# videolan/dav1d

Hardware: NVIDIA H100
Metric: Mpixels/s (higher is better)
Workload: dtype u8/i16->i32

## Files before the change

dav1d_b200/csrc/loopfilter.cu:

```cuda
#include "host_util.h"

namespace b200 {

template <bool HBD> struct LfMem {
    typename Bd<HBD>::pixel *p; ptrdiff_t sb;
    B200_DEV int get(int i) const { return p[i * sb]; }
    B200_DEV void set(int i, int v) { p[i * sb] = (typename Bd<HBD>::pixel)v; }
};
template <bool HBD, class Acc>
B200_DEV void lf_line_acc(Acc &px, int E, int I, int H, int wd, int bdmax)
{
    const int b8 = HBD ? (32 - __clz(bdmax)) - 8 : 0;
    const int F = 1 << b8;
    E <<= b8; I <<= b8; H <<= b8;
    const int p1 = px.get(-2), p0 = px.get(-1), q0 = px.get(0), q1 = px.get(1);
    int fm = iabs(p1 - p0) <= I && iabs(q1 - q0) <= I && iabs(p0 - q0) * 2 + (iabs(p1 - q1) >> 1) <= E;
    int p2 = 0, q2 = 0, p3 = 0, q3 = 0;
    if (wd > 4) {
        p2 = px.get(-3); q2 = px.get(2);
        fm &= iabs(p2 - p1) <= I && iabs(q2 - q1) <= I;
        if (wd > 6) {
            p3 = px.get(-4); q3 = px.get(3);
            fm &= iabs(p3 - p2) <= I && iabs(q3 - q2) <= I;
        }
    }
    if (!fm) return;
    int flat8in = 0;
    if (wd >= 6) flat8in = iabs(p2 - p0) <= F && iabs(p1 - p0) <= F && iabs(q1 - q0) <= F && iabs(q2 - q0) <= F;
    if (wd >= 8) flat8in &= iabs(p3 - p0) <= F && iabs(q3 - q0) <= F;
    if (wd >= 16) {
        const int p6 = px.get(-7), p5 = px.get(-6), p4 = px.get(-5), q4 = px.get(4), q5 = px.get(5), q6 = px.get(6);
        const int flat8out = iabs(p6 - p0) <= F && iabs(p5 - p0) <= F && iabs(p4 - p0) <= F &&
                             iabs(q4 - q0) <= F && iabs(q5 - q0) <= F && iabs(q6 - q0) <= F;
        if (flat8out & flat8in) {
            int s = p6 * 7 + p5 * 2 + p4 * 2 + p3 + p2 + p1 + p0 + q0 + 8;
            px.set(-6, (s >> 4)); s += -2 * p6 + p3 + q1;
            px.set(-5, (s >> 4)); s += -p6 - p5 + p2 + q2;
            px.set(-4, (s >> 4)); s += -p6 - p4 + p1 + q3;
            px.set(-3, (s >> 4)); s += -p6 - p3 + p0 + q4;
            px.set(-2, (s >> 4)); s += -p6 - p2 + q0 + q5;
            px.set(-1, (s >> 4)); s += -p6 - p1 + q1 + q6;
            px.set(0, (s >> 4)); s += -p5 - p0 + q2 + q6;
            px.set(1, (s >> 4)); s += -p4 - q0 + q3 + q6;
            px.set(2, (s >> 4)); s += -p3 - q1 + q4 + q6;
            px.set(3, (s >> 4)); s += -p2 - q2 + q5 + q6;
            px.set(4, (s >> 4)); s += -p1 - q3 + q6 + q6;
            px.set(5, (s >> 4));
            return;
        }
    }
    if (wd >= 8 && flat8in) {
        px.set(-3, ((p3 + p3 + p3 + 2 * p2 + p1 + p0 + q0 + 4) >> 3));
        px.set(-2, ((p3 + p3 + p2 + 2 * p1 + p0 + q0 + q1 + 4) >> 3));
        px.set(-1, ((p3 + p2 + p1 + 2 * p0 + q0 + q1 + q2 + 4) >> 3));
        px.set(0, ((p2 + p1 + p0 + 2 * q0 + q1 + q2 + q3 + 4) >> 3));
        px.set(1, ((p1 + p0 + q0 + 2 * q1 + q2 + q3 + q3 + 4) >> 3));
        px.set(2, ((p0 + q0 + q1 + 2 * q2 + q3 + q3 + q3 + 4) >> 3));
    } else if (wd == 6 && flat8in) {
        px.set(-2, ((p2 + 2 * p2 + 2 * p1 + 2 * p0 + q0 + 4) >> 3));
        px.set(-1, ((p2 + 2 * p1 + 2 * p0 + 2 * q0 + q1 + 4) >> 3));
        px.set(0, ((p1 + 2 * p0 + 2 * q0 + 2 * q1 + q2 + 4) >> 3));
        px.set(1, ((p0 + 2 * q0 + 2 * q1 + 2 * q2 + q2 + 4) >> 3));
    } else {
        const int lo = -128 * (1 << b8), hi = 128 * (1 << b8) - 1;
        const bool hev = iabs(p1 - p0) > H || iabs(q1 - q0) > H;
        int f = hev ? iclip(p1 - q1, lo, hi) : 0;
        f = iclip(3 * (q0 - p0) + f, lo, hi);
        const int f1 = imin(f + 4, hi) >> 3, f2 = imin(f + 3, hi) >> 3;
        px.set(-1, iclip(p0 + f2, 0, bdmax));
        px.set(0, iclip(q0 - f1, 0, bdmax));
        if (!hev) {
            const int g = (f1 + 1) >> 1;
            px.set(-2, iclip(p1 + g, 0, bdmax));
            px.set(1, iclip(q1 - g, 0, bdmax));
        }
    }
}

template <bool HBD>
B200_DEV void lf_line(typename Bd<HBD>::pixel *p, ptrdiff_t sb, int E, int I, int H, int wd, int bdmax)
{
    LfMem<HBD> m{ p, sb };
    lf_line_acc<HBD>(m, E, I, H, wd, bdmax);
}

B200_DEV int lf_width(const B200Av1Filter &m, int plane, int dir, int b, int a, int ss_a)
{
    if (plane == 0) {
        const int half = a >> 4, bit = a & 15;
        if ((m.filter_y[dir][b][2][half] >> bit) & 1) return 16;
        if ((m.filter_y[dir][b][1][half] >> bit) & 1) return 8;
        if ((m.filter_y[dir][b][0][half] >> bit) & 1) return 4;
        return 0;
    }
    const int hs = 16 >> ss_a;
    const int half = a >= hs, bit = a - half * hs;
    if ((m.filter_uv[dir][b][1][half] >> bit) & 1) return 6;
    if ((m.filter_uv[dir][b][0][half] >> bit) & 1) return 4;
    return 0;
}

template <bool HBD>
__global__ void __launch_bounds__(256) lf_cols_kernel(const __grid_constant__ B200LfFrame f, int bdmax, int ya4, int yb4)
{
    B200_PDL_ENTRY();
    typedef typename Bd<HBD>::pixel pixel;
    const int plane = blockIdx.z;
    if (plane ? !f.filter_uv : !f.filter_y) return;
    const int ssh = plane ? f.ss_hor : 0, ssv = plane ? f.ss_ver : 0;
    const int x4 = blockIdx.x * 32 + threadIdx.x;
    const int y4 = (ya4 >> ssv) + blockIdx.y * 8 + threadIdx.y;
    const int pw4 = (f.w4 + ssh) >> ssh, ph4 = imin((f.h4 + ssv) >> ssv, (yb4 + ssv) >> ssv);
    if (x4 >= pw4 || x4 == 0 || y4 >= ph4) return;
    const int sbx = x4 >> (5 - ssh), xi = x4 & ((32 >> ssh) - 1);
    const int sby = y4 >> (5 - ssv), yi = y4 & ((32 >> ssv) - 1);
    const B200Av1Filter &m = f.mask[sby * f.sb128w + sbx];
    const int wd = lf_width(m, plane, 0, xi, yi, ssv);
    if (!wd) return;
    const uint8_t (*l)[4] = f.level + (ptrdiff_t)y4 * f.b4_stride + x4;
    const int c = plane == 0 ? 0 : plane + 1;
    const int L = l[0][c] ? l[0][c] : l[-1][c];
    if (!L) return;
    const int E = f.lut.e[L], I = f.lut.i[L];
    pixel *p = (pixel *)f.pic + f.plane_off[plane] + (ptrdiff_t)(y4 * 4) * f.stride[plane] + x4 * 4;
#pragma unroll 1
    for (int k = 0; k < 4; k++, p += f.stride[plane]) lf_line<HBD>(p, 1, E, I, L >> 4, wd, bdmax);
}

template <bool HBD>
__global__ void __launch_bounds__(256) lf_rows_kernel(const __grid_constant__ B200LfFrame f, int bdmax, int ya4, int yb4)
{
    B200_PDL_ENTRY();
    typedef typename Bd<HBD>::pixel pixel;
    const int plane = blockIdx.z;
    if (plane ? !f.filter_uv : !f.filter_y) return;
    const int ssh = plane ? f.ss_hor : 0, ssv = plane ? f.ss_ver : 0;
    const int x = blockIdx.x * 128 + threadIdx.x;
    const int y4 = (ya4 >> ssv) + blockIdx.y * 2 + threadIdx.y;
    const int pw4 = (f.w4 + ssh) >> ssh, ph4 = imin((f.h4 + ssv) >> ssv, (yb4 + ssv) >> ssv);
    if (x >= pw4 * 4 || y4 >= ph4 || y4 == 0) return;
    const int x4 = x >> 2, sbx = x4 >> (5 - ssh), xi = x4 & ((32 >> ssh) - 1);
    const int sby = y4 >> (5 - ssv), yi = y4 & ((32 >> ssv) - 1);
    const B200Av1Filter &m = f.mask[sby * f.sb128w + sbx];
    const int wd = lf_width(m, plane, 1, yi, xi, ssh);
    if (!wd) return;
    const uint8_t (*l)[4] = f.level + (ptrdiff_t)y4 * f.b4_stride + x4;
    const int c = plane == 0 ? 1 : plane + 1;
    const int L = l[0][c] ? l[0][c] : l[-f.b4_stride][c];
    if (!L) return;
    pixel *p = (pixel *)f.pic + f.plane_off[plane] + (ptrdiff_t)(y4 * 4) * f.stride[plane] + x;
    lf_line<HBD>(p, f.stride[plane], f.lut.e[L], f.lut.i[L], L >> 4, wd, bdmax);
}

struct LfSbArgs {
    uint32_t mask[3];
    uint8_t cur[32], prev[32];
    B200FilterLUT lut;
    int plane_class, dir, n_units, stride;
};
template <bool HBD>
__global__ void lf_sb_kernel(typename Bd<HBD>::pixel *dst, LfSbArgs a, int bdmax)
{
    const int line = blockIdx.x * blockDim.x + threadIdx.x;
    if (line >= a.n_units * 4) return;
    const int u = line >> 2;
    int wd = 0;
    if (a.plane_class) wd = (a.mask[1] >> u) & 1 ? 6 : ((a.mask[0] >> u) & 1 ? 4 : 0);
    else wd = (a.mask[2] >> u) & 1 ? 16 : ((a.mask[1] >> u) & 1 ? 8 : ((a.mask[0] >> u) & 1 ? 4 : 0));
    if (!wd) return;
    const int L = a.cur[u] ? a.cur[u] : a.prev[u];
    if (!L) return;
    typename Bd<HBD>::pixel *p = a.dir ? dst + 8 * a.stride + line : dst + (ptrdiff_t)line * a.stride + 8;
    lf_line<HBD>(p, a.dir ? a.stride : 1, a.lut.e[L], a.lut.i[L], L >> 4, wd, bdmax);
}

int lf_frame_rows(int bdmax, const B200LfFrame *f, int ya4, int yb4, cudaStream_t stream)
{
    if (int r = check_bdmax(bdmax, "b200_lf_frame")) return r;
    if (!f->filter_y) return 0;
    ya4 = imax(ya4, 0); yb4 = imin(yb4, f->h4);
    if (yb4 <= ya4) return 0;
    if ((ya4 & 1) || ((yb4 & 1) && yb4 != f->h4)) { b200_set_error("b200_lf_frame: odd band boundary"); return -2; }
    const int w4 = f->w4, n4 = yb4 - ya4;
    if (int r = launch_hbd(bdmax, Launch::pdl, dim3((w4 + 31) / 32, (n4 + 7) / 8, 3), dim3(32, 8), 0, stream,
                           [&](auto hbd) { return std::make_tuple(lf_cols_kernel<hbd>, *f, bdmax, ya4, yb4); }))
        return r;
    return launch_hbd(bdmax, Launch::pdl, dim3((w4 * 4 + 127) / 128, (n4 + 1) / 2, 3), dim3(128, 2), 0, stream,
                      [&](auto hbd) { return std::make_tuple(lf_rows_kernel<hbd>, *f, bdmax, ya4, yb4); });
}

}

using namespace b200;

extern "C" {

int b200_lf_frame(int bdmax, const B200LfFrame *f, void *stream)
{
    return b200::lf_frame_rows(bdmax, f, 0, f->h4, (cudaStream_t)stream);
}

int b200_loop_filter_sb(int plane_class, int dir, void *dst, ptrdiff_t stride, const uint32_t *mask,
                        const uint8_t (*lvl)[4], ptrdiff_t lvl_stride, const B200FilterLUT *lut, int w, int bdmax)
{
    (void)w;
    if (int r = check_bdmax(bdmax, "b200_loop_filter_sb")) return r;
    const uint32_t vm = mask[0] | mask[1] | (plane_class ? 0 : mask[2]);
    if (!vm) return 0;
    int n_units = 32 - __builtin_clz(vm);
    Level1 L;
    const size_t px = bdmax > 255 ? 2 : 1;
    LfSbArgs a;
    memset(&a, 0, sizeof(a));
    a.mask[0] = mask[0]; a.mask[1] = mask[1]; a.mask[2] = plane_class ? 0 : mask[2];
    a.lut = *lut; a.plane_class = plane_class; a.dir = dir; a.n_units = n_units;
    for (int u = 0; u < n_units; u++) {
        const uint8_t (*l)[4] = lvl + (dir ? u : u * lvl_stride);
        a.cur[u] = l[0][0];
        a.prev[u] = dir ? l[-lvl_stride][0] : l[-1][0];
    }
    const int lines = n_units * 4;
    int ww, wh; uint8_t *org;
    if (dir) { ww = lines; wh = 16; org = (uint8_t *)dst - 8 * stride; }
    else { ww = 16; wh = lines; org = (uint8_t *)dst - 8 * (ptrdiff_t)px; }
    a.stride = ww;
    void *win = L.upload_rect(0, org, stride, ww, wh, px);
    if (!win) return -1;
    if (int r = launch_hbd(bdmax, Launch::plain, dim3((lines + 127) / 128), dim3(128), 0, 0,
                           [&](auto hbd) { return std::make_tuple(lf_sb_kernel<hbd>, (typename Bd<hbd>::pixel *)win, a, bdmax); }))
        return r;
    return L.download_rect(0, org, stride, ww, wh, px);
}

}

namespace {
template <int PC, int DIR> void lf8(uint8_t *d, ptrdiff_t s, const uint32_t *m, const uint8_t (*l)[4], ptrdiff_t ls, const B200FilterLUT *lut, int w) {
    if (b200_loop_filter_sb(PC, DIR, d, s, m, l, ls, lut, w, 255)) die("loop_filter_sb");
}
template <int PC, int DIR> void lf16(uint16_t *d, ptrdiff_t s, const uint32_t *m, const uint8_t (*l)[4], ptrdiff_t ls, const B200FilterLUT *lut, int w, int bd) {
    if (b200_loop_filter_sb(PC, DIR, d, s, m, l, ls, lut, w, bd)) die("loop_filter_sb");
}
}
extern "C" {
void b200_loop_filter_dsp_init_8bpc(B200LoopFilterDSPContext *c) {
    c->loop_filter_sb[0][0] = (void *)lf8<0, 0>; c->loop_filter_sb[0][1] = (void *)lf8<0, 1>;
    c->loop_filter_sb[1][0] = (void *)lf8<1, 0>; c->loop_filter_sb[1][1] = (void *)lf8<1, 1>;
}
void b200_loop_filter_dsp_init_16bpc(B200LoopFilterDSPContext *c) {
    c->loop_filter_sb[0][0] = (void *)lf16<0, 0>; c->loop_filter_sb[0][1] = (void *)lf16<0, 1>;
    c->loop_filter_sb[1][0] = (void *)lf16<1, 0>; c->loop_filter_sb[1][1] = (void *)lf16<1, 1>;
}
}
```

dav1d_b200/csrc/looprestoration.cu:

```cuda
#include "host_util.h"
#define B200_TBL __constant__
#include "tables_gen.h"

namespace b200 {

constexpr int kTW = 64, kTH = 32, kSW = kTW + 6, kSH = kTH + 6;

struct LrTileParams {
    int type;
    int fh[7], fv[7];
    unsigned s0, s1; int w0, w1;
};

struct LrShared {
    uint16_t src[kSH][kSW + 2];
    union {
        uint16_t hor[kSH][kTW];
        struct {
            int A3[kTH + 2][kTW + 2]; uint16_t B3[kTH + 2][kTW + 2];
            int A5[kTH / 2 + 2][kTW + 2]; uint16_t B5[kTH / 2 + 2][kTW + 2];
        } s;
    } u;
};

template <bool HBD, class Store>
B200_DEV void lr_tile_compute(LrShared &sm, const LrTileParams &P, int tw, int th, int bdmax, Store store)
{
    const int tid = threadIdx.x, nt = blockDim.x;
    const int bitdepth = HBD ? 32 - __clz(bdmax) : 8;
    if (P.type == 1) {
        const int rbh = 3 + (bitdepth == 12) * 2, rbv = 11 - (bitdepth == 12) * 2;
        const int clip_limit = 1 << (bitdepth + 1 + 7 - rbh);
        for (int i = tid; i < (th + 6) * (kTW / 4); i += nt) {
            const int y = i / (kTW / 4), x = (i - y * (kTW / 4)) * 4;
            if (x >= tw) continue;
            int v[10];
#pragma unroll
            for (int k = 0; k < 10; k++) v[k] = sm.src[y][x + k];
#pragma unroll
            for (int j = 0; j < 4; j++) {
                int sum = 1 << (bitdepth + 6);
                if (!HBD) sum += v[j + 3] * 128;
#pragma unroll
                for (int k = 0; k < 7; k++) sum += v[j + k] * P.fh[k];
                sm.u.hor[y][x + j] = (uint16_t)iclip((sum + (1 << (rbh - 1))) >> rbh, 0, clip_limit - 1);
            }
        }
        __syncthreads();
        const int round_offset = 1 << (bitdepth + (rbv - 1));
        for (int i = tid; i < ((th + 3) / 4) * kTW; i += nt) {
            const int yq = i / kTW, x = i - yq * kTW, y = yq * 4;
            if (x >= tw) continue;
            int v[10];
#pragma unroll
            for (int k = 0; k < 10; k++) v[k] = y + k < th + 6 ? (int)sm.u.hor[y + k][x] : 0;
#pragma unroll
            for (int j = 0; j < 4; j++) {
                if (y + j >= th) break;
                int sum = -round_offset;
#pragma unroll
                for (int k = 0; k < 7; k++) sum += v[j + k] * P.fv[k];
                store(x, y + j, iclip((sum + (1 << (rbv - 1))) >> rbv, 0, bdmax));
            }
        }
        return;
    }
    const int b8 = bitdepth - 8;
    if (P.s1) {
        constexpr int NS = (kTW + 2 + 3) / 4;
        for (int i = tid; i < (th + 2) * NS; i += nt) {
            const int yy = i / NS, xx = (i - yy * NS) * 4;
            if (xx >= tw + 2) continue;
            int cs[6], cq[6];
#pragma unroll
            for (int k = 0; k < 6; k++) {
                const int v0 = sm.src[yy + 1][xx + 1 + k], v1 = sm.src[yy + 2][xx + 1 + k], v2 = sm.src[yy + 3][xx + 1 + k];
                cs[k] = v0 + v1 + v2; cq[k] = v0 * v0 + v1 * v1 + v2 * v2;
            }
#pragma unroll
            for (int k = 0; k < 4; k++) {
                if (xx + k >= tw + 2) break;
                const int sum = cs[k] + cs[k + 1] + cs[k + 2], sq = cq[k] + cq[k + 1] + cq[k + 2];
                const int a = (sq + ((1 << (2 * b8)) >> 1)) >> (2 * b8);
                const int b = (sum + ((1 << b8) >> 1)) >> b8;
                const unsigned p = (unsigned)imax(a * 9 - b * b, 0);
                const unsigned z = (p * P.s1 + (1u << 19)) >> 20;
                const unsigned x = b200_sgr_x_by_x[z < 255u ? z : 255u];
                sm.u.s.A3[yy][xx + k] = (int)((x * (unsigned)sum * 455u + (1u << 11)) >> 12);
                sm.u.s.B3[yy][xx + k] = (uint16_t)x;
            }
        }
    }
    if (P.s0) {
        const int nrow = (th + 1) / 2 + 1;
        constexpr int NS = (kTW + 2 + 3) / 4;
        for (int i = tid; i < nrow * NS; i += nt) {
            const int j = i / NS, xx = (i - j * NS) * 4;
            if (xx >= tw + 2) continue;
            const int cy = 2 * j - 1 + 3;
            int cs[8], cq[8];
#pragma unroll
            for (int k = 0; k < 8; k++) {
                int su = 0, sq = 0;
#pragma unroll
                for (int dy = -2; dy <= 2; dy++) { const int v = sm.src[cy + dy][xx + k]; su += v; sq += v * v; }
                cs[k] = su; cq[k] = sq;
            }
#pragma unroll
            for (int k = 0; k < 4; k++) {
                if (xx + k >= tw + 2) break;
                const int sum = cs[k] + cs[k + 1] + cs[k + 2] + cs[k + 3] + cs[k + 4];
                const int sq = cq[k] + cq[k + 1] + cq[k + 2] + cq[k + 3] + cq[k + 4];
                const int a = (sq + ((1 << (2 * b8)) >> 1)) >> (2 * b8);
                const int b = (sum + ((1 << b8) >> 1)) >> b8;
                const unsigned p = (unsigned)imax(a * 25 - b * b, 0);
                const unsigned z = (p * P.s0 + (1u << 19)) >> 20;
                const unsigned x = b200_sgr_x_by_x[z < 255u ? z : 255u];
                sm.u.s.A5[j][xx + k] = (int)((x * (unsigned)sum * 164u + (1u << 11)) >> 12);
                sm.u.s.B5[j][xx + k] = (uint16_t)x;
            }
        }
    }
    __syncthreads();
    for (int i = tid; i < th * (kTW / 4); i += nt) {
        const int y = i / (kTW / 4), x = (i - y * (kTW / 4)) * 4;
        if (x >= tw) continue;
        int t5a[4] = { 0, 0, 0, 0 }, t5b[4] = { 0, 0, 0, 0 }, t3a[4] = { 0, 0, 0, 0 }, t3b[4] = { 0, 0, 0, 0 };
        if (P.s0) {
            int ca[6], cb[6];
            if (!(y & 1)) {
                const int j0 = y >> 1, j1 = j0 + 1;
#pragma unroll
                for (int k = 0; k < 6; k++) { ca[k] = (int)sm.u.s.B5[j0][x + k] + sm.u.s.B5[j1][x + k]; cb[k] = sm.u.s.A5[j0][x + k] + sm.u.s.A5[j1][x + k]; }
            } else {
                const int j = (y + 1) >> 1;
#pragma unroll
                for (int k = 0; k < 6; k++) { ca[k] = sm.u.s.B5[j][x + k]; cb[k] = sm.u.s.A5[j][x + k]; }
            }
#pragma unroll
            for (int k = 0; k < 4; k++) { t5a[k] = ca[k + 1] * 6 + (ca[k] + ca[k + 2]) * 5; t5b[k] = cb[k + 1] * 6 + (cb[k] + cb[k + 2]) * 5; }
        }
        if (P.s1) {
            const int ys = y + 1;
            int ma[6], va[6], mb[6], vb[6];
#pragma unroll
            for (int k = 0; k < 6; k++) {
                ma[k] = sm.u.s.B3[ys][x + k]; va[k] = (int)sm.u.s.B3[ys - 1][x + k] + sm.u.s.B3[ys + 1][x + k];
                mb[k] = sm.u.s.A3[ys][x + k]; vb[k] = sm.u.s.A3[ys - 1][x + k] + sm.u.s.A3[ys + 1][x + k];
            }
#pragma unroll
            for (int k = 0; k < 4; k++) {
                t3a[k] = (ma[k + 1] + ma[k] + ma[k + 2] + va[k + 1]) * 4 + (va[k] + va[k + 2]) * 3;
                t3b[k] = (mb[k + 1] + mb[k] + mb[k + 2] + vb[k + 1]) * 4 + (vb[k] + vb[k + 2]) * 3;
            }
        }
        int out[4];
#pragma unroll
        for (int k = 0; k < 4; k++) {
            const int src = sm.src[y + 3][x + k + 3];
            int t5 = 0, t3 = 0;
            if (P.s0) t5 = !(y & 1) ? (t5b[k] - t5a[k] * src + (1 << 8)) >> 9 : (t5b[k] - t5a[k] * src + (1 << 7)) >> 8;
            if (P.s1) t3 = (t3b[k] - t3a[k] * src + (1 << 8)) >> 9;
            const int v = P.w0 * t5 + P.w1 * t3;
            out[k] = iclip(src + ((v + (1 << 10)) >> 11), 0, bdmax);
        }
        store.row4(x, y, out, imin(4, tw - x));
    }
}

template <class pixel> struct LrStore {
    pixel *o; ptrdiff_t st;
    B200_DEV void operator()(int x, int y, int v) const { o[y * st + x] = (pixel)v; }
    B200_DEV void row4(int x, int y, const int (&v)[4], int n) const {
        pixel *p = o + y * st + x;
        if (n == 4 && !((uintptr_t)p & (4 * sizeof(pixel) - 1))) {
            if (sizeof(pixel) == 1) *(unsigned *)p = (unsigned)v[0] | (unsigned)v[1] << 8 | (unsigned)v[2] << 16 | (unsigned)v[3] << 24;
            else *(uint2 *)p = make_uint2((unsigned)v[0] | (unsigned)v[1] << 16, (unsigned)v[2] | (unsigned)v[3] << 16);
        } else {
#pragma unroll
            for (int k = 0; k < 4; k++) if (k < n) p[k] = (pixel)v[k];
        }
    }
};

B200_DEV void lr_unit_params(const B200RestorationUnit &u, bool hbd, LrTileParams &P)
{
    P.type = u.type == 0 ? 0 : (u.type == 2 ? 1 : 2);
    P.s0 = P.s1 = 0; P.w0 = P.w1 = 0;
    if (u.type == 2) {
#pragma unroll
        for (int i = 0; i < 3; i++) { P.fh[i] = P.fh[6 - i] = u.filter_h[i]; P.fv[i] = P.fv[6 - i] = u.filter_v[i]; }
        P.fh[3] = -(P.fh[0] + P.fh[1] + P.fh[2]) * 2 + (hbd ? 128 : 0);
        P.fv[3] = 128 - (P.fv[0] + P.fv[1] + P.fv[2]) * 2;
    } else if (u.type >= 3) {
        const int idx = u.type - 3;
        P.s0 = b200_sgr_params[idx][0]; P.s1 = b200_sgr_params[idx][1];
        P.w0 = u.sgr_weights[0]; P.w1 = 128 - (u.sgr_weights[0] + u.sgr_weights[1]);
        if (!P.s0) P.w0 = 0;
        if (!P.s1) P.w1 = 0;
    }
}

struct LrGrid { int base[3], nx[3]; unsigned nx_recip[3]; int ty0[3]; };

template <bool HBD>
#ifndef B200_LR_MINB
#define B200_LR_MINB 6
#endif
__global__ void __launch_bounds__(256, B200_LR_MINB) lr_frame_kernel(const __grid_constant__ B200LrFrame f, const __grid_constant__ LrGrid lg, int bdmax)
{
    B200_PDL_ENTRY();
    typedef typename Bd<HBD>::pixel pixel;
    __shared__ LrShared sm;
    const int bid = blockIdx.x;
    const int pl = bid >= lg.base[2] ? 2 : bid >= lg.base[1] ? 1 : 0;
    const int ssh = pl ? f.ss_hor : 0, ssv = pl ? f.ss_ver : 0;
    const int w = (f.w + ssh) >> ssh, h = (f.h + ssv) >> ssv;
    const int us_log2 = f.unit_size_log2[pl ? 1 : 0], unit = 1 << us_log2, half = unit >> 1;
    const int tw_full = unit < kTW ? unit : kTW;
    const int local = bid - lg.base[pl], nxp = lg.nx[pl];
    const int tyl = nxp > 1 ? (int)__umulhi((unsigned)local, lg.nx_recip[pl]) : local, txi = local - tyl * nxp;
    const int tyi = tyl + lg.ty0[pl];
    const int x0 = txi * tw_full;
    const int k = ssv ? tyi : tyi >> 1, ty = ssv ? 0 : tyi & 1;
    const int y0s = k ? (64 * k - 8) >> ssv : 0;
    const int y1s = imin(h, (64 * (k + 1) - 8) >> ssv);
    const int ty0 = y0s + ty * kTH;
    if (x0 >= w || y0s >= h || ty0 >= y1s) return;
    const int tw = imin(tw_full, w - x0), th = imin(kTH, y1s - ty0);
    const pixel *C = (const pixel *)f.cdef + f.plane_off[pl];
    const pixel *D = (const pixel *)f.dbl + f.plane_off[pl];
    pixel *O = (pixel *)f.dst + f.plane_off[pl];
    const int st = f.stride[pl];

    const bool have_top = y0s > 0, have_bot = y1s < h;
    constexpr int PPW = HBD ? 2 : 4;
    const bool interior = x0 >= 4 && x0 + tw + 4 <= w && !(tw & 3) && !(x0 & 3) && !(st & (PPW - 1)) &&
                          !(((uintptr_t)C | (uintptr_t)D | (uintptr_t)O) & 3);
    const int NW = (tw + 8) / PPW;
    const unsigned magic = recip16(NW);

    __shared__ LrTileParams sP;
    B200RestorationUnit u;
    u.type = 0;
    if (threadIdx.x == 0 && (f.restore_planes & (1 << pl))) {
        int n_full = 0;
        { const int max_unit = unit + half; if (w >= max_unit) n_full = (w - max_unit) / unit + 1; }
        const int ux = imin(x0 >> us_log2, n_full), xu = ux << us_log2;
        const int sby = ((y0s << ssv) + (y0s ? 8 : 0)) >> (6 + f.sb128);
        const int row_y = (sby << (6 + f.sb128)) >> ssv;
        int aligned = row_y & ~(unit - 1);
        if (aligned && aligned + half > h) aligned -= unit;
        aligned <<= ssv;
        const int sb_idx = (aligned >> 7) * f.sr_sb128w, unit_idx = ((aligned >> 6) & 1) << 1;
        const int shift_hor = 7 - ssh;
        u = f.lr_mask[sb_idx + (xu >> shift_hor)].lr[pl][unit_idx + ((xu >> (shift_hor - 1)) & 1)];
    }
    constexpr int NI = HBD ? 6 : 3;
    unsigned wv[NI];
    if (interior) {
#pragma unroll
        for (int n = 0; n < NI; n++) {
            const int i = threadIdx.x + n * 256;
            const int yy = (int)((i * magic) >> 16), g = i - yy * NW;
            if (yy >= th + 6) break;
            int Y = ty0 - 3 + yy;
            const pixel *base = C;
            if (Y < y0s) {
                if (have_top) { base = D; Y = imax(Y, y0s - 2); } else Y = y0s;
            } else if (Y >= y1s) {
                if (have_bot) { base = D; Y = imin(imin(Y, y1s + 1), h - 1); } else Y = y1s - 1;
            }
            wv[n] = *(const unsigned *)(base + (ptrdiff_t)Y * st + x0 - 4 + g * PPW);
        }
    }
    if (threadIdx.x == 0) {
        LrTileParams P;
        lr_unit_params(u, HBD, P);
        sP = P;
    }
    __syncthreads();
    const LrTileParams &P = sP;
    if (P.type == 0) {
        if (interior) {
#pragma unroll
            for (int n = 0; n < NI; n++) {
                const int i = threadIdx.x + n * 256;
                const int yy = (int)((i * magic) >> 16), g = i - yy * NW;
                if (yy >= th + 6) break;
                if (yy >= 3 && yy < th + 3 && g * PPW >= 4 && g * PPW < tw + 4)
                    *(unsigned *)(O + (ptrdiff_t)(ty0 - 3 + yy) * st + x0 - 4 + g * PPW) = wv[n];
            }
        } else
        for (int i = threadIdx.x; i < kTW * th; i += blockDim.x) {
            const int y = i / kTW, x = i - y * kTW;
            if (x >= tw) continue;
            O[(ptrdiff_t)(ty0 + y) * st + x0 + x] = C[(ptrdiff_t)(ty0 + y) * st + x0 + x];
        }
        return;
    }
    if (interior) {
#pragma unroll
        for (int n = 0; n < NI; n++) {
            const int i = threadIdx.x + n * 256;
            const int yy = (int)((i * magic) >> 16), g = i - yy * NW;
            if (yy >= th + 6) break;
            const int c0 = g * PPW - 1;
#pragma unroll
            for (int k = 0; k < PPW; k++) {
                const int c = c0 + k;
                if (c >= 0 && c < tw + 6) sm.src[yy][c] = (uint16_t)(HBD ? (wv[n] >> (16 * k)) & 0xffff : (wv[n] >> (8 * k)) & 0xff);
            }
        }
    } else
    for (int i = threadIdx.x; i < (th + 6) * kSW; i += blockDim.x) {
        const int yy = i / kSW, xx = i - yy * kSW;
        if (xx >= tw + 6) continue;
        int Y = ty0 - 3 + yy;
        const int X = iclip(x0 - 3 + xx, 0, w - 1);
        const pixel *base = C;
        if (Y < y0s) {
            if (have_top) { base = D; Y = imax(Y, y0s - 2); } else Y = y0s;
        } else if (Y >= y1s) {
            if (have_bot) { base = D; Y = imin(imin(Y, y1s + 1), h - 1); } else Y = y1s - 1;
        }
        sm.src[yy][xx] = base[(ptrdiff_t)Y * st + X];
    }
    __syncthreads();
    lr_tile_compute<HBD>(sm, P, tw, th, bdmax, LrStore<pixel>{ O + (ptrdiff_t)ty0 * st + x0, st });
}

template <bool HBD>
__global__ void __launch_bounds__(256) lr_window_kernel(const typename Bd<HBD>::pixel *win, typename Bd<HBD>::pixel *out,
                                                        int w, int h, LrTileParams P, int bdmax)
{
    __shared__ LrShared sm;
    const int x0 = blockIdx.x * kTW, y0 = blockIdx.y * kTH;
    const int tw = imin(kTW, w - x0), th = imin(kTH, h - y0);
    for (int i = threadIdx.x; i < (th + 6) * kSW; i += blockDim.x) {
        const int yy = i / kSW, xx = i - yy * kSW;
        if (xx >= tw + 6) continue;
        sm.src[yy][xx] = win[(size_t)(y0 + yy) * (w + 6) + x0 + xx];
    }
    __syncthreads();
    lr_tile_compute<HBD>(sm, P, tw, th, bdmax, LrStore<typename Bd<HBD>::pixel>{ out + (size_t)y0 * w + x0, w });
}

int lr_frame_rows(int bdmax, const B200LrFrame *f, int r0, int r1, cudaStream_t stream)
{
    if (int r = check_bdmax(bdmax, "b200_lr_frame")) return r;
    for (int i = 0; i < 2; i++)
        if (f->unit_size_log2[i] < 5 || f->unit_size_log2[i] > 8) { b200_set_error("b200_lr_frame: bad unit size"); return -2; }
    const int n_stripes = (f->h + 8 + 63) / 64;
    r0 = imax(r0, 0); r1 = imin(r1, 2 * n_stripes);
    LrGrid lg;
    int total = 0;
    for (int p = 0; p < 3; p++) {
        const int ssh = p ? f->ss_hor : 0, ssv = p ? f->ss_ver : 0;
        const int w = (f->w + ssh) >> ssh;
        const int unit = 1 << f->unit_size_log2[p ? 1 : 0], tw_full = unit < kTW ? unit : kTW;
        lg.nx[p] = (w + tw_full - 1) / tw_full;
        lg.nx_recip[p] = lg.nx[p] > 1 ? (unsigned)(((1ull << 32) + lg.nx[p] - 1) / lg.nx[p]) : 0u;
        lg.base[p] = total;
        const int a = ssv ? r0 >> 1 : r0, b = ssv ? r1 >> 1 : r1;
        lg.ty0[p] = a;
        total += lg.nx[p] * imax(b - a, 0);
    }
    if (!total) return 0;
    return launch_hbd(bdmax, Launch::pdl, dim3(total), dim3(256), 0, stream,
                      [&](auto hbd) { return std::make_tuple(lr_frame_kernel<hbd>, *f, lg, bdmax); });
}

}

using namespace b200;

extern "C" {

int b200_lr_frame(int bdmax, const B200LrFrame *f, void *stream)
{
    return b200::lr_frame_rows(bdmax, f, 0, 1 << 30, (cudaStream_t)stream);
}

int b200_lr_filter(int kind, void *dst, ptrdiff_t stride, const void *left, const void *lpf, int w, int h,
                   const void *params, int edges, int bdmax)
{
    if (int r = check_bdmax(bdmax, "b200_lr_filter")) return r;
    if (kind < 0 || kind > 3 || w < 1 || w > 384 || h < 1 || h > 64) { b200_set_error("b200_lr_filter: bad arguments"); return -2; }
    Level1 L;
    const size_t px = bdmax > 255 ? 2 : 1;
    int use_bottom;
    if (kind == 0) use_bottom = (edges & 8) && h > ((edges & 4) ? 3 : 5);
    else if (kind == 2) use_bottom = (edges & 8) && h > 2;
    else use_bottom = (edges & 8) && !(h & 1) && h > ((edges & 4) ? 2 : 4);
    uint8_t *win = (uint8_t *)L.host((size_t)(w + 6) * (h + 6) * px);
    if (!win) return -1;
    for (int y = -3; y < h + 3; y++) {
        const uint8_t *row; int from_unit = 0, yy = y;
        if (y < 0 && (edges & 4)) row = (const uint8_t *)lpf + (ptrdiff_t)((y < -2 ? -2 : y) + 2) * stride;
        else if (y >= h && use_bottom) row = (const uint8_t *)lpf + (ptrdiff_t)(6 + (y - h > 1 ? 1 : y - h)) * stride;
        else { yy = y < 0 ? 0 : y >= h ? h - 1 : y; row = (const uint8_t *)dst + (ptrdiff_t)yy * stride; from_unit = 1; }
        for (int x = -3; x < w + 3; x++) {
            const uint8_t *sp;
            if (x < 0) {
                if (!(edges & 1)) sp = row;
                else if (from_unit && left) sp = (const uint8_t *)left + ((size_t)yy * 4 + 4 + x) * px;
                else sp = row + (ptrdiff_t)x * (ptrdiff_t)px;
            } else if (x >= w && !(edges & 2)) sp = row + (size_t)(w - 1) * px;
            else sp = row + (size_t)x * px;
            memcpy(win + ((size_t)(y + 3) * (w + 6) + (x + 3)) * px, sp, px);
        }
    }
    LrTileParams P;
    memset(&P, 0, sizeof(P));
    if (kind == 0) {
        const int16_t (*flt)[8] = (const int16_t (*)[8])params;
        P.type = 1;
        for (int i = 0; i < 7; i++) { P.fh[i] = flt[0][i]; P.fv[i] = flt[1][i]; }
    } else {
        const uint32_t *sp = (const uint32_t *)params;
        const int16_t *wp = (const int16_t *)(sp + 2);
        P.type = 2;
        P.s0 = kind == 2 ? 0 : sp[0]; P.s1 = kind == 1 ? 0 : sp[1];
        P.w0 = kind == 2 ? 0 : wp[0]; P.w1 = kind == 1 ? 0 : wp[1];
        if (kind == 1) P.w0 = wp[0];
    }
    void *in, *out;
    if (!(in = L.upload(0, win, (size_t)(w + 6) * (h + 6) * px)) || !(out = L.dev(1, (size_t)w * h * px))) return -1;
    if (int r = launch_hbd(bdmax, Launch::plain, dim3((w + kTW - 1) / kTW, (h + kTH - 1) / kTH), dim3(256), 0, 0, [&](auto hbd) {
            typedef typename Bd<hbd>::pixel pixel;
            return std::make_tuple(lr_window_kernel<hbd>, (const pixel *)in, (pixel *)out, w, h, P, bdmax);
        }))
        return r;
    return L.download_rect(1, dst, stride, w, h, px);
}

}

namespace {
template <int K> void lr8(uint8_t *d, ptrdiff_t s, const void *l, const uint8_t *lpf, int w, int h, const void *p, int e) {
    if (b200_lr_filter(K, d, s, l, lpf, w, h, p, e, 255)) die("looprestoration");
}
template <int K> void lr16(uint16_t *d, ptrdiff_t s, const void *l, const uint16_t *lpf, int w, int h, const void *p, int e, int bd) {
    if (b200_lr_filter(K, d, s, l, lpf, w, h, p, e, bd)) die("looprestoration");
}
}
extern "C" {
void b200_loop_restoration_dsp_init_8bpc(B200LoopRestorationDSPContext *c, int bpc) {
    (void)bpc;
    c->wiener[0] = c->wiener[1] = (void *)lr8<0>;
    c->sgr[0] = (void *)lr8<1>; c->sgr[1] = (void *)lr8<2>; c->sgr[2] = (void *)lr8<3>;
}
void b200_loop_restoration_dsp_init_16bpc(B200LoopRestorationDSPContext *c, int bpc) {
    (void)bpc;
    c->wiener[0] = c->wiener[1] = (void *)lr16<0>;
    c->sgr[0] = (void *)lr16<1>; c->sgr[1] = (void *)lr16<2>; c->sgr[2] = (void *)lr16<3>;
}
}
```

Baseline: 22500.

## Vectorize row loop filter to 4-pixel words and compact per-plane grid

The horizontal-edge (rows) kernel now has one thread per 4x4 block edge instead of one per pixel column. Each thread loads packed 4-sample words (u32 for 8-bit, uint2 for high bit depth), filters the four columns in registers, and writes the words back only if some column was filtered. Both kernels move from a fixed 3-plane grid to a flattened 1D grid sized to each plane's actual (subsampled) extent, so chroma CTAs that do nothing are no longer launched. This adds a 4-sample alignment requirement on strides and offsets, more registers per thread, and per-block plane decoding.

After: 23500, median of 6. +4.5%, better.

```diff
diff --git a/dav1d_b200/csrc/loopfilter.cu b/dav1d_b200/csrc/loopfilter.cu
--- a/dav1d_b200/csrc/loopfilter.cu
+++ b/dav1d_b200/csrc/loopfilter.cu
@@ -8,7 +8,7 @@
     B200_DEV void set(int i, int v) { p[i * sb] = (typename Bd<HBD>::pixel)v; }
 };
 template <bool HBD, class Acc>
-B200_DEV void lf_line_acc(Acc &px, int E, int I, int H, int wd, int bdmax)
+B200_DEV int lf_line_acc(Acc &px, int E, int I, int H, int wd, int bdmax)
 {
     const int b8 = HBD ? (32 - __clz(bdmax)) - 8 : 0;
     const int F = 1 << b8;
@@ -24,7 +24,7 @@
             fm &= iabs(p3 - p2) <= I && iabs(q3 - q2) <= I;
         }
     }
-    if (!fm) return;
+    if (!fm) return 0;
     int flat8in = 0;
     if (wd >= 6) flat8in = iabs(p2 - p0) <= F && iabs(p1 - p0) <= F && iabs(q1 - q0) <= F && iabs(q2 - q0) <= F;
     if (wd >= 8) flat8in &= iabs(p3 - p0) <= F && iabs(q3 - q0) <= F;
@@ -46,7 +46,7 @@
             px.set(3, (s >> 4)); s += -p2 - q2 + q5 + q6;
             px.set(4, (s >> 4)); s += -p1 - q3 + q6 + q6;
             px.set(5, (s >> 4));
-            return;
+            return 1;
         }
     }
     if (wd >= 8 && flat8in) {
@@ -75,6 +75,7 @@
             px.set(1, iclip(q1 - g, 0, bdmax));
         }
     }
+    return 1;
 }
 
 template <bool HBD>
@@ -82,6 +83,51 @@
 {
     LfMem<HBD> m{ p, sb };
     lf_line_acc<HBD>(m, E, I, H, wd, bdmax);
+}
+
+template <bool HBD> struct LfWord;
+template <> struct LfWord<false> {
+    typedef uint32_t T;
+    static B200_DEV int get(T w, int c) { return (w >> (8 * c)) & 0xff; }
+    static B200_DEV void set(T &w, int c, int v) { w = (w & ~(0xffu << (8 * c))) | ((unsigned)v << (8 * c)); }
+};
+template <> struct LfWord<true> {
+    typedef uint2 T;
+    static B200_DEV int get(T w, int c) { return ((c & 2 ? w.y : w.x) >> (16 * (c & 1))) & 0xffff; }
+    static B200_DEV void set(T &w, int c, int v)
+    {
+        unsigned &h = c & 2 ? w.y : w.x;
+        h = (h & ~(0xffffu << (16 * (c & 1)))) | ((unsigned)v << (16 * (c & 1)));
+    }
+};
+template <bool HBD, int C> struct LfCol {
+    typename LfWord<HBD>::T *r;
+    B200_DEV int get(int i) const { return LfWord<HBD>::get(r[i + 7], C); }
+    B200_DEV void set(int i, int v) { LfWord<HBD>::set(r[i + 7], C, v); }
+};
+
+struct LfPlaneGrid { int pw4, y0, ph4, gx, n; };
+B200_HD LfPlaneGrid lf_plane_grid(const B200LfFrame &f, int plane, int ya4, int yb4)
+{
+    const int ssh = plane ? f.ss_hor : 0, ssv = plane ? f.ss_ver : 0;
+    LfPlaneGrid g;
+    g.pw4 = (f.w4 + ssh) >> ssh;
+    g.y0 = ya4 >> ssv;
+    g.ph4 = imin((f.h4 + ssv) >> ssv, (yb4 + ssv) >> ssv);
+    g.gx = (g.pw4 + 31) >> 5;
+    g.n = g.gx * ((g.ph4 - g.y0 + 7) >> 3);
+    return g;
+}
+B200_DEV bool lf_thread_unit(const B200LfFrame &f, int ya4, int yb4, int &plane, int &x4, int &y4)
+{
+    int b = blockIdx.x;
+    plane = 0;
+    LfPlaneGrid g = lf_plane_grid(f, 0, ya4, yb4);
+    while (b >= g.n) { b -= g.n; g = lf_plane_grid(f, ++plane, ya4, yb4); }
+    const int by = b / g.gx, bx = b - by * g.gx;
+    x4 = bx * 32 + threadIdx.x;
+    y4 = g.y0 + by * 8 + threadIdx.y;
+    return x4 < g.pw4 && y4 < g.ph4;
 }
 
 B200_DEV int lf_width(const B200Av1Filter &m, int plane, int dir, int b, int a, int ss_a)
@@ -105,13 +151,9 @@
 {
     B200_PDL_ENTRY();
     typedef typename Bd<HBD>::pixel pixel;
-    const int plane = blockIdx.z;
-    if (plane ? !f.filter_uv : !f.filter_y) return;
+    int plane, x4, y4;
+    if (!lf_thread_unit(f, ya4, yb4, plane, x4, y4) || x4 == 0) return;
     const int ssh = plane ? f.ss_hor : 0, ssv = plane ? f.ss_ver : 0;
-    const int x4 = blockIdx.x * 32 + threadIdx.x;
-    const int y4 = (ya4 >> ssv) + blockIdx.y * 8 + threadIdx.y;
-    const int pw4 = (f.w4 + ssh) >> ssh, ph4 = imin((f.h4 + ssv) >> ssv, (yb4 + ssv) >> ssv);
-    if (x4 >= pw4 || x4 == 0 || y4 >= ph4) return;
     const int sbx = x4 >> (5 - ssh), xi = x4 & ((32 >> ssh) - 1);
     const int sby = y4 >> (5 - ssv), yi = y4 & ((32 >> ssv) - 1);
     const B200Av1Filter &m = f.mask[sby * f.sb128w + sbx];
@@ -132,14 +174,11 @@
 {
     B200_PDL_ENTRY();
     typedef typename Bd<HBD>::pixel pixel;
-    const int plane = blockIdx.z;
-    if (plane ? !f.filter_uv : !f.filter_y) return;
+    typedef typename LfWord<HBD>::T word;
+    int plane, x4, y4;
+    if (!lf_thread_unit(f, ya4, yb4, plane, x4, y4) || y4 == 0) return;
     const int ssh = plane ? f.ss_hor : 0, ssv = plane ? f.ss_ver : 0;
-    const int x = blockIdx.x * 128 + threadIdx.x;
-    const int y4 = (ya4 >> ssv) + blockIdx.y * 2 + threadIdx.y;
-    const int pw4 = (f.w4 + ssh) >> ssh, ph4 = imin((f.h4 + ssv) >> ssv, (yb4 + ssv) >> ssv);
-    if (x >= pw4 * 4 || y4 >= ph4 || y4 == 0) return;
-    const int x4 = x >> 2, sbx = x4 >> (5 - ssh), xi = x4 & ((32 >> ssh) - 1);
+    const int sbx = x4 >> (5 - ssh), xi = x4 & ((32 >> ssh) - 1);
     const int sby = y4 >> (5 - ssv), yi = y4 & ((32 >> ssv) - 1);
     const B200Av1Filter &m = f.mask[sby * f.sb128w + sbx];
     const int wd = lf_width(m, plane, 1, yi, xi, ssh);
@@ -148,8 +187,25 @@
     const int c = plane == 0 ? 1 : plane + 1;
     const int L = l[0][c] ? l[0][c] : l[-f.b4_stride][c];
     if (!L) return;
-    pixel *p = (pixel *)f.pic + f.plane_off[plane] + (ptrdiff_t)(y4 * 4) * f.stride[plane] + x;
-    lf_line<HBD>(p, f.stride[plane], f.lut.e[L], f.lut.i[L], L >> 4, wd, bdmax);
+    const int E = f.lut.e[L], I = f.lut.i[L], H = L >> 4;
+    const ptrdiff_t s = f.stride[plane] >> 2;
+    word *p = (word *)((pixel *)f.pic + f.plane_off[plane] + (ptrdiff_t)(y4 * 4) * f.stride[plane] + x4 * 4);
+    const int nr = wd == 16 ? 7 : wd == 8 ? 4 : wd == 6 ? 3 : 2;
+    word r[14];
+#pragma unroll
+    for (int k = 0; k < 14; k++)
+        if (k >= 7 - nr && k < 7 + nr) r[k] = p[(k - 7) * s];
+    LfCol<HBD, 0> c0{ r };
+    LfCol<HBD, 1> c1{ r };
+    LfCol<HBD, 2> c2{ r };
+    LfCol<HBD, 3> c3{ r };
+    const int fm = lf_line_acc<HBD>(c0, E, I, H, wd, bdmax) | lf_line_acc<HBD>(c1, E, I, H, wd, bdmax) |
+                   lf_line_acc<HBD>(c2, E, I, H, wd, bdmax) | lf_line_acc<HBD>(c3, E, I, H, wd, bdmax);
+    if (!fm) return;
+    const int nw = wd == 16 ? 6 : wd == 8 ? 3 : 2;
+#pragma unroll
+    for (int k = 1; k < 13; k++)
+        if (k >= 7 - nw && k < 7 + nw) p[(k - 7) * s] = r[k];
 }
 
 struct LfSbArgs {
@@ -178,14 +234,19 @@
 {
     if (int r = check_bdmax(bdmax, "b200_lf_frame")) return r;
     if (!f->filter_y) return 0;
+    const int planes = f->filter_uv ? 3 : 1;
+    const size_t px = bdmax > 255 ? 2 : 1;
+    for (int pl = 0; pl < planes; pl++)
+        if ((f->stride[pl] & 3) || (f->plane_off[pl] & 3) || ((uintptr_t)f->pic % (4 * px))) { b200_set_error("b200_lf_frame: planes must be 4-sample aligned"); return -2; }
     ya4 = imax(ya4, 0); yb4 = imin(yb4, f->h4);
     if (yb4 <= ya4) return 0;
     if ((ya4 & 1) || ((yb4 & 1) && yb4 != f->h4)) { b200_set_error("b200_lf_frame: odd band boundary"); return -2; }
-    const int w4 = f->w4, n4 = yb4 - ya4;
-    if (int r = launch_hbd(bdmax, Launch::pdl, dim3((w4 + 31) / 32, (n4 + 7) / 8, 3), dim3(32, 8), 0, stream,
+    int ctas = 0;
+    for (int pl = 0; pl < planes; pl++) ctas += lf_plane_grid(*f, pl, ya4, yb4).n;
+    if (int r = launch_hbd(bdmax, Launch::pdl, dim3(ctas), dim3(32, 8), 0, stream,
                            [&](auto hbd) { return std::make_tuple(lf_cols_kernel<hbd>, *f, bdmax, ya4, yb4); }))
         return r;
-    return launch_hbd(bdmax, Launch::pdl, dim3((w4 * 4 + 127) / 128, (n4 + 1) / 2, 3), dim3(128, 2), 0, stream,
+    return launch_hbd(bdmax, Launch::pdl, dim3(ctas), dim3(32, 8), 0, stream,
                       [&](auto hbd) { return std::make_tuple(lf_rows_kernel<hbd>, *f, bdmax, ya4, yb4); });
 }
 
```

## Pair chroma tiles per block and stage SGR lookup table in shared memory

Applied to the files above, without the earlier changes.

When the chroma unit size is 32, each 256-thread block now runs two 32-wide chroma tiles (U and V) at once, with two 128-thread halves and separate shared-memory slices, and the V-plane blocks are dropped from the grid. This is meant to cut the idle threads and extra blocks that narrow chroma tiles cause. The x_by_x table moves from constant memory into a shared-memory copy, so divergent lookups no longer serialize on the constant cache. Type-0 copy tiles now go through the shared source tile instead of storing directly, and the tile compute is split into two passes, which adds a table-staging step to every block.

Result: faster. 22490 before, 23260 after (median of 6 runs) (+3.4%).

```diff
diff --git a/dav1d_b200/csrc/looprestoration.cu b/dav1d_b200/csrc/looprestoration.cu
--- a/dav1d_b200/csrc/looprestoration.cu
+++ b/dav1d_b200/csrc/looprestoration.cu
@@ -1,38 +1,51 @@
 #include "host_util.h"
-#define B200_TBL __constant__
+#define B200_TBL __device__
 #include "tables_gen.h"
 
 namespace b200 {
 
-constexpr int kTW = 64, kTH = 32, kSW = kTW + 6, kSH = kTH + 6;
+constexpr int kTW = 64, kTH = 32, kSH = kTH + 6;
 
 struct LrTileParams {
     int type;
     int fh[7], fv[7];
     unsigned s0, s1; int w0, w1;
+    ptrdiff_t out; int st;
 };
 
-struct LrShared {
-    uint16_t src[kSH][kSW + 2];
+template <int TW> struct LrShared {
+    static constexpr int SW = TW + 6;
+    LrTileParams P;
+    uint16_t src[kSH][SW + 2];
     union {
-        uint16_t hor[kSH][kTW];
+        uint16_t hor[kSH][TW];
         struct {
-            int A3[kTH + 2][kTW + 2]; uint16_t B3[kTH + 2][kTW + 2];
-            int A5[kTH / 2 + 2][kTW + 2]; uint16_t B5[kTH / 2 + 2][kTW + 2];
+            int A3[kTH + 2][TW + 2]; uint16_t B3[kTH + 2][TW + 2];
+            int A5[kTH / 2 + 2][TW + 2]; uint16_t B5[kTH / 2 + 2][TW + 2];
         } s;
     } u;
 };
-
-template <bool HBD, class Store>
-B200_DEV void lr_tile_compute(LrShared &sm, const LrTileParams &P, int tw, int th, int bdmax, Store store)
-{
-    const int tid = threadIdx.x, nt = blockDim.x;
+constexpr size_t kLrSmem = sizeof(LrShared<kTW>) > 2 * sizeof(LrShared<32>) ? sizeof(LrShared<kTW>) : 2 * sizeof(LrShared<32>);
+
+B200_DEV void lr_stage_x_by_x(unsigned *tbl)
+{
+    const int i = threadIdx.x;
+    if (i < 64)
+        tbl[i] = (unsigned)b200_sgr_x_by_x[4 * i] | (unsigned)b200_sgr_x_by_x[4 * i + 1] << 8 |
+                 (unsigned)b200_sgr_x_by_x[4 * i + 2] << 16 | (unsigned)b200_sgr_x_by_x[4 * i + 3] << 24;
+}
+
+template <bool HBD, int TW>
+B200_DEV void lr_tile_pass1(LrShared<TW> &sm, const LrTileParams &P, const unsigned *tbl, int tw, int th, int bdmax,
+                            int tid, int nt)
+{
     const int bitdepth = HBD ? 32 - __clz(bdmax) : 8;
+    const uint8_t *x_by_x = (const uint8_t *)tbl;
     if (P.type == 1) {
-        const int rbh = 3 + (bitdepth == 12) * 2, rbv = 11 - (bitdepth == 12) * 2;
+        const int rbh = 3 + (bitdepth == 12) * 2;
         const int clip_limit = 1 << (bitdepth + 1 + 7 - rbh);
-        for (int i = tid; i < (th + 6) * (kTW / 4); i += nt) {
-            const int y = i / (kTW / 4), x = (i - y * (kTW / 4)) * 4;
+        for (int i = tid; i < (th + 6) * (TW / 4); i += nt) {
+            const int y = i / (TW / 4), x = (i - y * (TW / 4)) * 4;
             if (x >= tw) continue;
             int v[10];
 #pragma unroll
@@ -46,28 +59,11 @@
                 sm.u.hor[y][x + j] = (uint16_t)iclip((sum + (1 << (rbh - 1))) >> rbh, 0, clip_limit - 1);
             }
         }
-        __syncthreads();
-        const int round_offset = 1 << (bitdepth + (rbv - 1));
-        for (int i = tid; i < ((th + 3) / 4) * kTW; i += nt) {
-            const int yq = i / kTW, x = i - yq * kTW, y = yq * 4;
-            if (x >= tw) continue;
-            int v[10];
-#pragma unroll
-            for (int k = 0; k < 10; k++) v[k] = y + k < th + 6 ? (int)sm.u.hor[y + k][x] : 0;
-#pragma unroll
-            for (int j = 0; j < 4; j++) {
-                if (y + j >= th) break;
-                int sum = -round_offset;
-#pragma unroll
-                for (int k = 0; k < 7; k++) sum += v[j + k] * P.fv[k];
-                store(x, y + j, iclip((sum + (1 << (rbv - 1))) >> rbv, 0, bdmax));
-            }
-        }
         return;
     }
     const int b8 = bitdepth - 8;
+    constexpr int NS = (TW + 2 + 3) / 4;
     if (P.s1) {
-        constexpr int NS = (kTW + 2 + 3) / 4;
         for (int i = tid; i < (th + 2) * NS; i += nt) {
             const int yy = i / NS, xx = (i - yy * NS) * 4;
             if (xx >= tw + 2) continue;
@@ -85,7 +81,7 @@
                 const int b = (sum + ((1 << b8) >> 1)) >> b8;
                 const unsigned p = (unsigned)imax(a * 9 - b * b, 0);
                 const unsigned z = (p * P.s1 + (1u << 19)) >> 20;
-                const unsigned x = b200_sgr_x_by_x[z < 255u ? z : 255u];
+                const unsigned x = x_by_x[z < 255u ? z : 255u];
                 sm.u.s.A3[yy][xx + k] = (int)((x * (unsigned)sum * 455u + (1u << 11)) >> 12);
                 sm.u.s.B3[yy][xx + k] = (uint16_t)x;
             }
@@ -93,7 +89,6 @@
     }
     if (P.s0) {
         const int nrow = (th + 1) / 2 + 1;
-        constexpr int NS = (kTW + 2 + 3) / 4;
         for (int i = tid; i < nrow * NS; i += nt) {
             const int j = i / NS, xx = (i - j * NS) * 4;
             if (xx >= tw + 2) continue;
@@ -115,15 +110,40 @@
                 const int b = (sum + ((1 << b8) >> 1)) >> b8;
                 const unsigned p = (unsigned)imax(a * 25 - b * b, 0);
                 const unsigned z = (p * P.s0 + (1u << 19)) >> 20;
-                const unsigned x = b200_sgr_x_by_x[z < 255u ? z : 255u];
+                const unsigned x = x_by_x[z < 255u ? z : 255u];
                 sm.u.s.A5[j][xx + k] = (int)((x * (unsigned)sum * 164u + (1u << 11)) >> 12);
                 sm.u.s.B5[j][xx + k] = (uint16_t)x;
             }
         }
     }
-    __syncthreads();
-    for (int i = tid; i < th * (kTW / 4); i += nt) {
-        const int y = i / (kTW / 4), x = (i - y * (kTW / 4)) * 4;
+}
+
+template <bool HBD, int TW, class Store>
+B200_DEV void lr_tile_pass2(LrShared<TW> &sm, const LrTileParams &P, int tw, int th, int bdmax, int tid, int nt, Store store)
+{
+    const int bitdepth = HBD ? 32 - __clz(bdmax) : 8;
+    if (P.type == 1) {
+        const int rbv = 11 - (bitdepth == 12) * 2;
+        const int round_offset = 1 << (bitdepth + (rbv - 1));
+        for (int i = tid; i < ((th + 3) / 4) * TW; i += nt) {
+            const int yq = i / TW, x = i - yq * TW, y = yq * 4;
+            if (x >= tw) continue;
+            int v[10];
+#pragma unroll
+            for (int k = 0; k < 10; k++) v[k] = y + k < th + 6 ? (int)sm.u.hor[y + k][x] : 0;
+#pragma unroll
+            for (int j = 0; j < 4; j++) {
+                if (y + j >= th) break;
+                int sum = -round_offset;
+#pragma unroll
+                for (int k = 0; k < 7; k++) sum += v[j + k] * P.fv[k];
+                store(x, y + j, iclip((sum + (1 << (rbv - 1))) >> rbv, 0, bdmax));
+            }
+        }
+        return;
+    }
+    for (int i = tid; i < th * (TW / 4); i += nt) {
+        const int y = i / (TW / 4), x = (i - y * (TW / 4)) * 4;
         if (x >= tw) continue;
         int t5a[4] = { 0, 0, 0, 0 }, t5b[4] = { 0, 0, 0, 0 }, t3a[4] = { 0, 0, 0, 0 }, t3b[4] = { 0, 0, 0, 0 };
         if (P.s0) {
@@ -201,26 +221,20 @@
     }
 }
 
-struct LrGrid { int base[3], nx[3]; unsigned nx_recip[3]; int ty0[3]; };
-
-template <bool HBD>
-#ifndef B200_LR_MINB
-#define B200_LR_MINB 6
-#endif
-__global__ void __launch_bounds__(256, B200_LR_MINB) lr_frame_kernel(const __grid_constant__ B200LrFrame f, const __grid_constant__ LrGrid lg, int bdmax)
-{
-    B200_PDL_ENTRY();
+struct LrGrid { int base[3], nx[3]; unsigned nx_recip[3]; int ty0[3]; int pair; };
+
+template <bool HBD, int TW, int NT>
+B200_DEV void lr_frame_tile(const B200LrFrame &f, const LrGrid &lg, int bdmax, int rp, int pl, int local, int tid,
+                            LrShared<TW> &sm, const unsigned *tbl)
+{
     typedef typename Bd<HBD>::pixel pixel;
-    __shared__ LrShared sm;
-    const int bid = blockIdx.x;
-    const int pl = bid >= lg.base[2] ? 2 : bid >= lg.base[1] ? 1 : 0;
     const int ssh = pl ? f.ss_hor : 0, ssv = pl ? f.ss_ver : 0;
     const int w = (f.w + ssh) >> ssh, h = (f.h + ssv) >> ssv;
     const int us_log2 = f.unit_size_log2[pl ? 1 : 0], unit = 1 << us_log2, half = unit >> 1;
-    const int tw_full = unit < kTW ? unit : kTW;
-    const int local = bid - lg.base[pl], nxp = lg.nx[pl];
-    const int tyl = nxp > 1 ? (int)__umulhi((unsigned)local, lg.nx_recip[pl]) : local, txi = local - tyl * nxp;
-    const int tyi = tyl + lg.ty0[pl];
+    const int tw_full = unit < TW ? unit : TW;
+    const int nxp = lg.nx[rp];
+    const int tyl = nxp > 1 ? (int)__umulhi((unsigned)local, lg.nx_recip[rp]) : local, txi = local - tyl * nxp;
+    const int tyi = tyl + lg.ty0[rp];
     const int x0 = txi * tw_full;
     const int k = ssv ? tyi : tyi >> 1, ty = ssv ? 0 : tyi & 1;
     const int y0s = k ? (64 * k - 8) >> ssv : 0;
@@ -230,20 +244,18 @@
     const int tw = imin(tw_full, w - x0), th = imin(kTH, y1s - ty0);
     const pixel *C = (const pixel *)f.cdef + f.plane_off[pl];
     const pixel *D = (const pixel *)f.dbl + f.plane_off[pl];
-    pixel *O = (pixel *)f.dst + f.plane_off[pl];
     const int st = f.stride[pl];
 
     const bool have_top = y0s > 0, have_bot = y1s < h;
     constexpr int PPW = HBD ? 2 : 4;
     const bool interior = x0 >= 4 && x0 + tw + 4 <= w && !(tw & 3) && !(x0 & 3) && !(st & (PPW - 1)) &&
-                          !(((uintptr_t)C | (uintptr_t)D | (uintptr_t)O) & 3);
+                          !(((uintptr_t)C | (uintptr_t)D | (uintptr_t)((pixel *)f.dst + f.plane_off[pl])) & 3);
     const int NW = (tw + 8) / PPW;
     const unsigned magic = recip16(NW);
 
-    __shared__ LrTileParams sP;
     B200RestorationUnit u;
     u.type = 0;
-    if (threadIdx.x == 0 && (f.restore_planes & (1 << pl))) {
+    if (tid == 0 && (f.restore_planes & (1 << pl))) {
         int n_full = 0;
         { const int max_unit = unit + half; if (w >= max_unit) n_full = (w - max_unit) / unit + 1; }
         const int ux = imin(x0 >> us_log2, n_full), xu = ux << us_log2;
@@ -256,12 +268,12 @@
         const int shift_hor = 7 - ssh;
         u = f.lr_mask[sb_idx + (xu >> shift_hor)].lr[pl][unit_idx + ((xu >> (shift_hor - 1)) & 1)];
     }
-    constexpr int NI = HBD ? 6 : 3;
+    constexpr int NI = ((kSH * (TW + 8)) / PPW + NT - 1) / NT;
     unsigned wv[NI];
     if (interior) {
 #pragma unroll
         for (int n = 0; n < NI; n++) {
-            const int i = threadIdx.x + n * 256;
+            const int i = tid + n * NT;
             const int yy = (int)((i * magic) >> 16), g = i - yy * NW;
             if (yy >= th + 6) break;
             int Y = ty0 - 3 + yy;
@@ -274,35 +286,10 @@
             wv[n] = *(const unsigned *)(base + (ptrdiff_t)Y * st + x0 - 4 + g * PPW);
         }
     }
-    if (threadIdx.x == 0) {
-        LrTileParams P;
-        lr_unit_params(u, HBD, P);
-        sP = P;
-    }
-    __syncthreads();
-    const LrTileParams &P = sP;
-    if (P.type == 0) {
-        if (interior) {
-#pragma unroll
-            for (int n = 0; n < NI; n++) {
-                const int i = threadIdx.x + n * 256;
-                const int yy = (int)((i * magic) >> 16), g = i - yy * NW;
-                if (yy >= th + 6) break;
-                if (yy >= 3 && yy < th + 3 && g * PPW >= 4 && g * PPW < tw + 4)
-                    *(unsigned *)(O + (ptrdiff_t)(ty0 - 3 + yy) * st + x0 - 4 + g * PPW) = wv[n];
-            }
-        } else
-        for (int i = threadIdx.x; i < kTW * th; i += blockDim.x) {
-            const int y = i / kTW, x = i - y * kTW;
-            if (x >= tw) continue;
-            O[(ptrdiff_t)(ty0 + y) * st + x0 + x] = C[(ptrdiff_t)(ty0 + y) * st + x0 + x];
-        }
-        return;
-    }
     if (interior) {
 #pragma unroll
         for (int n = 0; n < NI; n++) {
-            const int i = threadIdx.x + n * 256;
+            const int i = tid + n * NT;
             const int yy = (int)((i * magic) >> 16), g = i - yy * NW;
             if (yy >= th + 6) break;
             const int c0 = g * PPW - 1;
@@ -313,8 +300,8 @@
             }
         }
     } else
-    for (int i = threadIdx.x; i < (th + 6) * kSW; i += blockDim.x) {
-        const int yy = i / kSW, xx = i - yy * kSW;
+    for (int i = tid; i < (th + 6) * LrShared<TW>::SW; i += NT) {
+        const int yy = i / LrShared<TW>::SW, xx = i - yy * LrShared<TW>::SW;
         if (xx >= tw + 6) continue;
         int Y = ty0 - 3 + yy;
         const int X = iclip(x0 - 3 + xx, 0, w - 1);
@@ -326,24 +313,66 @@
         }
         sm.src[yy][xx] = base[(ptrdiff_t)Y * st + X];
     }
+    if (tid == 0) {
+        LrTileParams P;
+        lr_unit_params(u, HBD, P);
+        P.out = f.plane_off[pl] + (ptrdiff_t)ty0 * st + x0; P.st = st;
+        sm.P = P;
+    }
     __syncthreads();
-    lr_tile_compute<HBD>(sm, P, tw, th, bdmax, LrStore<pixel>{ O + (ptrdiff_t)ty0 * st + x0, st });
+    const LrTileParams &P = sm.P;
+    if (P.type == 0) {
+        const LrStore<pixel> store{ (pixel *)f.dst + P.out, P.st };
+        for (int i = tid; i < th * (TW / 4); i += NT) {
+            const int y = i / (TW / 4), x = (i - y * (TW / 4)) * 4;
+            if (x >= tw) continue;
+            const int v[4] = { sm.src[y + 3][x + 3], sm.src[y + 3][x + 4], sm.src[y + 3][x + 5], sm.src[y + 3][x + 6] };
+            store.row4(x, y, v, imin(4, tw - x));
+        }
+    } else
+        lr_tile_pass1<HBD>(sm, P, tbl, tw, th, bdmax, tid, NT);
+    __syncthreads();
+    if (P.type) lr_tile_pass2<HBD>(sm, P, tw, th, bdmax, tid, NT, LrStore<pixel>{ (pixel *)f.dst + P.out, P.st });
+}
+
+template <bool HBD>
+#ifndef B200_LR_MINB
+#define B200_LR_MINB 6
+#endif
+__global__ void __launch_bounds__(256, B200_LR_MINB) lr_frame_kernel(const __grid_constant__ B200LrFrame f, const __grid_constant__ LrGrid lg, int bdmax)
+{
+    B200_PDL_ENTRY();
+    __shared__ __align__(16) unsigned char smem[kLrSmem];
+    __shared__ unsigned tbl[64];
+    lr_stage_x_by_x(tbl);
+    const int bid = blockIdx.x;
+    const int pl = bid >= lg.base[2] ? 2 : bid >= lg.base[1] ? 1 : 0;
+    if (pl && lg.pair) {
+        const int hf = threadIdx.x >> 7;
+        lr_frame_tile<HBD, 32, 128>(f, lg, bdmax, 1, 1 + hf, bid - lg.base[1], threadIdx.x & 127,
+                                    ((LrShared<32> *)smem)[hf], tbl);
+    } else
+        lr_frame_tile<HBD, kTW, 256>(f, lg, bdmax, pl, pl, bid - lg.base[pl], threadIdx.x, *(LrShared<kTW> *)smem, tbl);
 }
 
 template <bool HBD>
 __global__ void __launch_bounds__(256) lr_window_kernel(const typename Bd<HBD>::pixel *win, typename Bd<HBD>::pixel *out,
                                                         int w, int h, LrTileParams P, int bdmax)
 {
-    __shared__ LrShared sm;
+    __shared__ LrShared<kTW> sm;
+    __shared__ unsigned tbl[64];
+    lr_stage_x_by_x(tbl);
     const int x0 = blockIdx.x * kTW, y0 = blockIdx.y * kTH;
     const int tw = imin(kTW, w - x0), th = imin(kTH, h - y0);
-    for (int i = threadIdx.x; i < (th + 6) * kSW; i += blockDim.x) {
-        const int yy = i / kSW, xx = i - yy * kSW;
+    for (int i = threadIdx.x; i < (th + 6) * LrShared<kTW>::SW; i += blockDim.x) {
+        const int yy = i / LrShared<kTW>::SW, xx = i - yy * LrShared<kTW>::SW;
         if (xx >= tw + 6) continue;
         sm.src[yy][xx] = win[(size_t)(y0 + yy) * (w + 6) + x0 + xx];
     }
     __syncthreads();
-    lr_tile_compute<HBD>(sm, P, tw, th, bdmax, LrStore<typename Bd<HBD>::pixel>{ out + (size_t)y0 * w + x0, w });
+    lr_tile_pass1<HBD>(sm, P, tbl, tw, th, bdmax, (int)threadIdx.x, (int)blockDim.x);
+    __syncthreads();
+    lr_tile_pass2<HBD>(sm, P, tw, th, bdmax, (int)threadIdx.x, (int)blockDim.x, LrStore<typename Bd<HBD>::pixel>{ out + (size_t)y0 * w + x0, w });
 }
 
 int lr_frame_rows(int bdmax, const B200LrFrame *f, int r0, int r1, cudaStream_t stream)
@@ -354,6 +383,7 @@
     const int n_stripes = (f->h + 8 + 63) / 64;
     r0 = imax(r0, 0); r1 = imin(r1, 2 * n_stripes);
     LrGrid lg;
+    lg.pair = f->unit_size_log2[1] == 5;
     int total = 0;
     for (int p = 0; p < 3; p++) {
         const int ssh = p ? f->ss_hor : 0, ssv = p ? f->ss_ver : 0;
@@ -364,7 +394,7 @@
         lg.base[p] = total;
         const int a = ssv ? r0 >> 1 : r0, b = ssv ? r1 >> 1 : r1;
         lg.ty0[p] = a;
-        total += lg.nx[p] * imax(b - a, 0);
+        if (p < 2 || !lg.pair) total += lg.nx[p] * imax(b - a, 0);
     }
     if (!total) return 0;
     return launch_hbd(bdmax, Launch::pdl, dim3(total), dim3(256), 0, stream,
```
